# vincenthz/eccoxide

Hardware: AMD Instinct MI355X
Metric: variable-base scalarmuls/sec (batch) per GPU + achieved HBM GB/s vs roofline (higher is better)
Workload: dtype u32

## Files before the change

### __graft_entry__.py

```python
import os
import subprocess
import sys

ROOT = os.path.dirname(os.path.abspath(__file__))
if ROOT not in sys.path:
    sys.path.insert(0, ROOT)


def build() -> None:
    jobs = str(min(6, os.cpu_count() or 1))
    subprocess.check_call(["make", "-C", os.path.join(ROOT, "eccoxide_amd", "csrc"), "-j", jobs, "ARCH=gfx950"])
    subprocess.check_call(["make", "-C", os.path.join(ROOT, "oracle")])
    subprocess.check_call(["make", "-C", os.path.join(ROOT, "tests", "cpp")])
    subprocess.check_call(["make", "-C", os.path.join(ROOT, "tests", "hip")])
    subprocess.check_call(["make", "-C", os.path.join(ROOT, "tests", "hip_p256k1")])
    subprocess.check_call(["make", "-C", os.path.join(ROOT, "tests", "hip_merged")])
    import eccoxide_amd
    from eccoxide_amd import _lib

    lib = _lib.load()
    assert lib.eccx_field_bytes(eccoxide_amd.P256R1) == 32


def smoke() -> None:
    import eccoxide_amd as E
    from eccoxide_amd import workload as W
    from tests import oracle_lib

    ora = oracle_lib.load()
    with E.Engine(0) as eng:
        for curve, n in (("p256r1", 300), ("ed25519", 300)):
# ... 41 lines not shown
```

### eccoxide_amd/csrc/ufe.hpp

```cpp
#pragma once
#include "fe.hpp"

#ifndef ECCX_SOLINAS_REDUCE
#define ECCX_SOLINAS_REDUCE 1
#endif

namespace eccx {

#include "umad_chunks.inc"

__device__ __forceinline__ void smad1_k(uint64_t& acc, uint32_t a, int32_t k) {
  asm("v_mad_i64_i32 %0, vcc, %1, %2, %0" : "+v"(acc) : "v"(a), "s"(k) : "vcc");
}

__device__ __forceinline__ void smad1_v(uint64_t& acc, int32_t a, int32_t b) {
  asm("v_mad_i64_i32 %0, vcc, %1, %2, %0" : "+v"(acc) : "v"(a), "v"(b) : "vcc");
}

enum : int { UK_MONT_PP1 = 0, UK_MONT = 1, UK_MERSENNE = 2, UK_PM19 = 3 };

template <class C, int K, int V>
struct U {
  static_assert(K >= 1 && K < (1 << (32 - C::B)), "limb bound out of range (limbs must stay below 2^32)");
  static_assert(V >= 1 && V <= 4096, "value bound out of range");
  uint32_t v[C::N];
};

template <class C>
struct UB {
  static constexpr bool MONT = C::KIND == UK_MONT_PP1 || C::KIND == UK_MONT;
  static constexpr bool WRAPPED = C::KIND == UK_MERSENNE;
  static constexpr int KMAX = (1 << (32 - C::B)) - 1;
  static constexpr uint64_t COL = (uint64_t)1 << (2 * C::B);
  static constexpr bool SPARSE = C::KIND == UK_MONT_PP1 && C::SPARSE_N > 0;
  static constexpr int KKMAX = WRAPPED  ? (int)(~(uint64_t)0 / ((uint64_t)(2 * C::N - 1) * COL))
                               : SPARSE ? (int)((~(uint64_t)0 >> 1) / ((uint64_t)C::N * COL)) - 1
                                        : (int)(~(uint64_t)0 / ((uint64_t)C::N * COL)) - 1;
  static_assert(KKMAX >= 1, "limbs too wide for this many columns");
  static constexpr bool kk_ok(int k1, int k2) { return k1 * k2 <= KKMAX; }
  static constexpr int KSQ_SHIFT = WRAPPED ? 2 : 1;
  static constexpr bool ksq_ok(int k) { return k * k <= KKMAX && (k << KSQ_SHIFT) <= KMAX + 1; }
  static constexpr int vout(int v1, int v2) {
    return MONT ? (int)(((uint32_t)(v1 * v2) + C::RP - 1) / C::RP) + 1 : (C::KIND == UK_PM19 ? 2 : 3);
  }
  static constexpr int KLAZY = ksq_ok(2) ? 2 : 1;
};

template <bool KC>
struct UMacQ {
  uint32_t x[9], y[9];
  int n = 0;
  ECCX_DEV void push(uint64_t& acc, uint32_t a, uint32_t b) {
    x[n] = a;
    y[n] = b;
    if (++n == 9) flush(acc);
  }
  ECCX_DEV void flush(uint64_t& acc) {
#define ECCX_Q(i) x[i], y[i]
    if constexpr (KC) {
      switch (n) {
// ... 15 lines not shown
        case 3: umad3_v(acc, ECCX_Q(0), ECCX_Q(1), ECCX_Q(2)); break;
        case 4: umad4_v(acc, ECCX_Q(0), ECCX_Q(1), ECCX_Q(2), ECCX_Q(3)); break;
        case 5: umad5_v(acc, ECCX_Q(0), ECCX_Q(1), ECCX_Q(2), ECCX_Q(3), ECCX_Q(4)); break;
        case 6: umad6_v(acc, ECCX_Q(0), ECCX_Q(1), ECCX_Q(2), ECCX_Q(3), ECCX_Q(4), ECCX_Q(5)); break;
        case 7: umad7_v(acc, ECCX_Q(0), ECCX_Q(1), ECCX_Q(2), ECCX_Q(3), ECCX_Q(4), ECCX_Q(5), ECCX_Q(6)); break;
        case 8: umad8_v(acc, ECCX_Q(0), ECCX_Q(1), ECCX_Q(2), ECCX_Q(3), ECCX_Q(4), ECCX_Q(5), ECCX_Q(6), ECCX_Q(7)); break;
        case 9: umad9_v(acc, ECCX_Q(0), ECCX_Q(1), ECCX_Q(2), ECCX_Q(3), ECCX_Q(4), ECCX_Q(5), ECCX_Q(6), ECCX_Q(7), ECCX_Q(8)); break;
        default: break;
      }
    }
#undef ECCX_Q
    n = 0;
  }
};


template <class C, bool SQR, bool BCONST>
ECCX_DEV void u_mul_core_mont(uint32_t (&r)[C::N], const uint32_t (&a)[C::N], const uint32_t (&b)[C::N]) {
  constexpr int N = C::N;
  constexpr bool PP1 = C::KIND == UK_MONT_PP1;
  auto PR = [](int j) constexpr { return PP1 ? C::PP1[j] : C::P[j]; };
  uint32_t m[N], t[N], a2[N];
  if constexpr (SQR) {
#pragma unroll
    for (int i = 0; i < N; ++i) a2[i] = a[i] << 1;
  }
  uint64_t acc = 0;
  UMacQ<BCONST> qa;
  UMacQ<true> qm;
#pragma unroll
  for (int k = 0; k < 2 * N - 1; ++k) {
    const int lo = k < N ? 0 : k - N + 1, hi = k < N ? k : N - 1;
    if constexpr (SQR) {
#pragma unroll
      for (int i = lo; 2 * i < k; ++i) qa.push(acc, a[i], a2[k - i]);
      if ((k & 1) == 0) qa.push(acc, a[k / 2], a[k / 2]);
    } else {
#pragma unroll
      for (int i = lo; i <= hi; ++i) qa.push(acc, a[i], b[k - i]);
    }
    qa.flush(acc);
    if constexpr (UB<C>::SPARSE) {
#pragma unroll
// ... 5 lines not shown
      }
      qm.flush(acc);
#pragma unroll
      for (int t = 0; t < C::SPARSE_N; ++t) {
        const int i = k - C::SPARSE_OFF[t];
        if (i >= lo && i <= (k < N ? k - 1 : N - 1)) {
          if (C::SPARSE_SIGN[t] < 0) smad1_k(acc, m[i], -(int32_t)(1u << C::SPARSE_SHIFT[t]));
        }
      }
    } else {
#pragma unroll
      for (int i = lo; i <= (k < N ? k - 1 : N - 1); ++i) {
        if (PR(k - i) != 0) qm.push(acc, m[i], PR(k - i));
      }
      qm.flush(acc);
    }
    if (k < N) {
      if constexpr (PP1) {
        m[k] = (uint32_t)acc & C::MASK;
      } else {
        m[k] = ((uint32_t)acc * C::N0B) & C::MASK;
        umad1_k(acc, m[k], C::P[0]);
      }
    } else {
      t[k - N] = (uint32_t)acc & C::MASK;
    }
    if constexpr (UB<C>::SPARSE) acc = (uint64_t)((int64_t)acc >> C::B);
    else acc >>= C::B;
  }
  t[N - 1] = (uint32_t)acc;
// ... 138 lines not shown
  t[N - 1] = (uint32_t)acc;
#pragma unroll
  for (int i = 0; i < N; ++i) r[i] = t[i];
}

template <class C, bool NEG_SQ>
ECCX_DEV void u_mul_sub_core_pp1(uint32_t (&r)[C::N], const uint32_t (&a)[C::N], const uint32_t (&b)[C::N],
                                 const uint32_t (&c)[C::N], const uint32_t (&d)[C::N]) {
  constexpr int N = C::N;
  static_assert(C::KIND == UK_MONT_PP1 && C::SPARSE_N == 0, "p = -1 mod 2^B with p + 1 as plain digits");
  uint32_t m[N], t[N];
  int32_t nc[N];
#pragma unroll
  for (int i = 0; i < N; ++i) nc[i] = NEG_SQ ? -(int32_t)(c[i] << 1) : -(int32_t)c[i];
  uint64_t acc = 0;
  UMacQ<false> qa;
  UMacQ<true> qm;
#pragma unroll
  for (int k = 0; k < 2 * N - 1; ++k) {
    const int lo = k < N ? 0 : k - N + 1, hi = k < N ? k : N - 1;
    if (k >= N && C::P[k - N] != 0) acc += (uint64_t)C::P[k - N];
#pragma unroll
    for (int i = lo; i <= hi; ++i) qa.push(acc, a[i], b[k - i]);
    qa.flush(acc);
    if constexpr (NEG_SQ) {
#pragma unroll
      for (int i = lo; 2 * i < k; ++i) smad1_v(acc, nc[i], (int32_t)(c[k - i] << 1));
      if ((k & 1) == 0) smad1_v(acc, nc[k / 2], (int32_t)c[k / 2]);
    } else {
#pragma unroll
      for (int i = lo; i <= hi; ++i) smad1_v(acc, nc[i], (int32_t)d[k - i]);
    }
#pragma unroll
    for (int i = lo; i <= (k < N ? k - 1 : N - 1); ++i) {
      if (C::PP1[k - i] != 0) qm.push(acc, m[i], C::PP1[k - i]);
    }
    qm.flush(acc);
    if (k < N) m[k] = (uint32_t)acc & C::MASK;
    else t[k - N] = (uint32_t)acc & C::MASK;
    acc = (uint64_t)((int64_t)acc >> C::B);
  }
  acc += (uint64_t)C::P[N - 1];
  t[N - 1] = (uint32_t)acc;
#pragma unroll
  for (int i = 0; i < N; ++i) r[i] = t[i];
}

template <class C, bool SQR, bool BCONST>
ECCX_DEV void u_mul_core_mers(uint32_t (&r)[C::N], const uint32_t (&a)[C::N], const uint32_t (&b)[C::N]) {
  constexpr int N = C::N;
  constexpr int S = C::B * N - C::PBITS;
  static_assert(S >= 1 && S <= 2, "wrap factor must keep shifted limbs below 2^32");
// ... 200 lines not shown
ECCX_DEV auto u_mul_add(const U<C, K1, V1>& a, const U<C, K2, V2>& b, const U<C, K3, V3>& c, const U<C, K4, V4>& d) {
  static_assert(C::KIND == UK_MONT, "merged products are implemented for the general Montgomery fields");
  static_assert(K1 * K2 + K3 * K4 <= UB<C>::KKMAX, "two products overflow the columns: reduce an operand first");
  constexpr int VO = (int)(((uint32_t)(V1 * V2 + V3 * V4) + C::RP - 1) / C::RP) + 1;
  static_assert(VO <= 3, "result too large: reduce an operand first");
  U<C, 1, VO> r;
  u_mul2_core_mont<C>(r.v, a.v, b.v, c.v, d.v);
  return r;
}

template <class C>
struct UBS {
  static constexpr bool OK = UB<C>::SPARSE || C::KIND == UK_MONT;
  static constexpr bool DENSE = C::KIND == UK_MONT_PP1 && !UB<C>::SPARSE;
  static constexpr int KKS = (int)((~(uint64_t)0 >> 1) / ((uint64_t)C::N * UB<C>::COL)) - 1;
  static constexpr bool ks_ok(int k) { return ((uint64_t)(k + 1) << C::B) <= ((uint64_t)1 << 31); }
};

template <class C, int K1, int V1, int K2, int V2, int K3, int V3, int K4, int V4>
ECCX_DEV auto u_mul_sub(const U<C, K1, V1>& a, const U<C, K2, V2>& b, const U<C, K3, V3>& c, const U<C, K4, V4>& d) {
  static_assert(UBS<C>::OK || UBS<C>::DENSE, "implemented for the Montgomery fields with room for signed columns");
  static_assert(K1 * K2 <= UBS<C>::KKS && K3 * K4 <= UBS<C>::KKS, "a product overflows the signed columns");
  static_assert(UBS<C>::ks_ok(K3) && UBS<C>::ks_ok(K4), "negated / signed operands must stay below 2^31");
  static_assert((uint32_t)(V1 * V2) < C::RP && (uint32_t)(V3 * V4) < C::RP, "result outside (0, 3p)");
  U<C, 1, 3> r;
  if constexpr (UB<C>::SPARSE) u_mul_sub_core_sparse<C, false>(r.v, a.v, b.v, c.v, d.v);
  else if constexpr (UBS<C>::DENSE) u_mul_sub_core_pp1<C, false>(r.v, a.v, b.v, c.v, d.v);
  else u_mul_sub_core_mont<C, false>(r.v, a.v, b.v, c.v, d.v);
  return r;
}
// ... 20 lines not shown
    return r;
  }
}

template <class C, int K1, int V1>
ECCX_DEV auto u_mul_k(const U<C, K1, V1>& a, const uint32_t (&k)[C::N]) {
  if constexpr (!UB<C>::kk_ok(K1, 1) || (UB<C>::vout(V1, 1) > 3)) {
    return u_mul_k(u_reduce(a), k);
  } else {
    U<C, 1, UB<C>::vout(V1, 1)> r;
    u_mul_core<C, false, true>(r.v, a.v, k);
    return r;
  }
}

template <class C, int K1, int V1>
ECCX_DEV U<C, 1, 2> u_mul_small(const U<C, K1, V1>& a, uint32_t k) {
  static_assert(C::KIND == UK_PM19, "written for 2^255 - 19");
  constexpr int N = C::N;
  uint32_t t[N];
  uint64_t acc = 0;
#pragma unroll
  for (int i = 0; i < N; ++i) {
    umad1_v(acc, a.v[i], k);
    t[i] = (uint32_t)acc & C::MASK;
    acc >>= C::B;
  }
  u_pm_tail<C>(t, acc);
  U<C, 1, 2> r;
#pragma unroll
// ... 162 lines not shown
}

template <class C>
ECCX_DEV U<C, 1, 2> u_to_mont(const Fe<C::Sat::L>& plain) {
  if constexpr (UB<C>::MONT) return u_as<1, 2>(u_mul_k<C>(u_from_sat<C>(plain), C::R2));
  else return u_from_sat<C>(plain);
}

template <class C, int K, int V>
ECCX_DEV void u_to_canonical(Fe<C::Sat::L>& out, const U<C, K, V>& a) {
  Fe<C::Sat::L> s;
  if constexpr (UB<C>::MONT) {
    uint32_t one[C::N];
#pragma unroll
    for (int i = 0; i < C::N; ++i) one[i] = (i == 0) ? 1u : 0u;
    auto r = u_mul_k<C>(u_reduce(a), one);
    u_to_sat<C>(s, r);
  } else {
    auto r = u_reduce(u_reduce(a));
    u_to_sat<C>(s, r);
  }
  uint32_t t[C::Sat::L];
#pragma unroll
  for (int i = 0; i < C::Sat::L; ++i) t[i] = s.v[i];
  cond_sub_p<typename C::Sat>(out, t, 0u);
}

template <class C, int K, int V>
ECCX_DEV void u_to_sat_mont(Fe<C::Sat::L>& out, const U<C, K, V>& a) {
  if constexpr (UB<C>::MONT) {
    auto r = u_mul_k<C>(u_reduce(a), C::RS);
    Fe<C::Sat::L> s;
    u_to_sat<C>(s, r);
    uint32_t t[C::Sat::L];
#pragma unroll
    for (int i = 0; i < C::Sat::L; ++i) t[i] = s.v[i];
    cond_sub_p<typename C::Sat>(out, t, 0u);
  } else {
    u_to_canonical<C>(out, a);
  }
}

}
```

### eccoxide_amd/csrc/umad_chunks.inc

```
__device__ __forceinline__ void umad1_v(uint64_t& acc, uint32_t a0, uint32_t b0) {
  asm("v_mad_u64_u32 %0, vcc, %1, %2, %0\n\t"
      : "+v"(acc)
      : "v"(a0), "v"(b0)
      : "vcc");
}
__device__ __forceinline__ void umad2_v(uint64_t& acc, uint32_t a0, uint32_t b0, uint32_t a1, uint32_t b1) {
  asm("v_mad_u64_u32 %0, vcc, %1, %2, %0\n\t"
      "v_mad_u64_u32 %0, vcc, %3, %4, %0\n\t"
      : "+v"(acc)
      : "v"(a0), "v"(b0), "v"(a1), "v"(b1)
      : "vcc");
}
__device__ __forceinline__ void umad3_v(uint64_t& acc, uint32_t a0, uint32_t b0, uint32_t a1, uint32_t b1, uint32_t a2, uint32_t b2) {
  asm("v_mad_u64_u32 %0, vcc, %1, %2, %0\n\t"
      "v_mad_u64_u32 %0, vcc, %3, %4, %0\n\t"
      "v_mad_u64_u32 %0, vcc, %5, %6, %0\n\t"
      : "+v"(acc)
      : "v"(a0), "v"(b0), "v"(a1), "v"(b1), "v"(a2), "v"(b2)
      : "vcc");
}
__device__ __forceinline__ void umad4_v(uint64_t& acc, uint32_t a0, uint32_t b0, uint32_t a1, uint32_t b1, uint32_t a2, uint32_t b2, uint32_t a3, uint32_t b3) {
  asm("v_mad_u64_u32 %0, vcc, %1, %2, %0\n\t"
      "v_mad_u64_u32 %0, vcc, %3, %4, %0\n\t"
      "v_mad_u64_u32 %0, vcc, %5, %6, %0\n\t"
// ... 140 lines not shown
}
__device__ __forceinline__ void umad9_k(uint64_t& acc, uint32_t a0, uint32_t b0, uint32_t a1, uint32_t b1, uint32_t a2, uint32_t b2, uint32_t a3, uint32_t b3, uint32_t a4, uint32_t b4, uint32_t a5, uint32_t b5, uint32_t a6, uint32_t b6, uint32_t a7, uint32_t b7, uint32_t a8, uint32_t b8) {
  asm("v_mad_u64_u32 %0, vcc, %1, %2, %0\n\t"
      "v_mad_u64_u32 %0, vcc, %3, %4, %0\n\t"
      "v_mad_u64_u32 %0, vcc, %5, %6, %0\n\t"
      "v_mad_u64_u32 %0, vcc, %7, %8, %0\n\t"
      "v_mad_u64_u32 %0, vcc, %9, %10, %0\n\t"
      "v_mad_u64_u32 %0, vcc, %11, %12, %0\n\t"
      "v_mad_u64_u32 %0, vcc, %13, %14, %0\n\t"
      "v_mad_u64_u32 %0, vcc, %15, %16, %0\n\t"
      "v_mad_u64_u32 %0, vcc, %17, %18, %0\n\t"
      : "+v"(acc)
      : "v"(a0), "s"(b0), "v"(a1), "s"(b1), "v"(a2), "s"(b2), "v"(a3), "s"(b3), "v"(a4), "s"(b4), "v"(a5), "s"(b5), "v"(a6), "s"(b6), "v"(a7), "s"(b7), "v"(a8), "s"(b8)
      : "vcc");
}
```

Baseline: 73.56 million.

## Use full 32-bit Montgomery digits and fold carry into next MAD chain

For dense p+1-form Montgomery fields, the low Montgomery digits m[k] become the full low 32 bits of the accumulator instead of B-bit masked values. The high half is carried forward by a multiply-by-2^S that is fused as the first MAD of the next column's chain, which removes the separate mask, shift and carry instructions per column. New static asserts bound column overflow, and the output value bound changes. Conversion out of Montgomery form keeps the old path through a dedicated exit multiply. This trades more inline-asm variants and looser bounds for fewer ALU ops in the inner multiply.

```diff
diff --git a/__graft_entry__.py b/__graft_entry__.py
--- a/__graft_entry__.py
+++ b/__graft_entry__.py
@@ -15,6 +15,7 @@
     subprocess.check_call(["make", "-C", os.path.join(ROOT, "tests", "hip")])
     subprocess.check_call(["make", "-C", os.path.join(ROOT, "tests", "hip_p256k1")])
     subprocess.check_call(["make", "-C", os.path.join(ROOT, "tests", "hip_merged")])
+    subprocess.check_call(["make", "-C", os.path.join(ROOT, "tests", "hip_lo32")])
     import eccoxide_amd
     from eccoxide_amd import _lib
 
diff --git a/eccoxide_amd/csrc/ufe.hpp b/eccoxide_amd/csrc/ufe.hpp
--- a/eccoxide_amd/csrc/ufe.hpp
+++ b/eccoxide_amd/csrc/ufe.hpp
@@ -1,5 +1,7 @@
 #pragma once
 #include "fe.hpp"
+
+#include <type_traits>
 
 #ifndef ECCX_SOLINAS_REDUCE
 #define ECCX_SOLINAS_REDUCE 1
@@ -15,6 +17,19 @@
 
 __device__ __forceinline__ void smad1_v(uint64_t& acc, int32_t a, int32_t b) {
   asm("v_mad_i64_i32 %0, vcc, %1, %2, %0" : "+v"(acc) : "v"(a), "v"(b) : "vcc");
+}
+
+template <int S>
+__device__ __forceinline__ void ucarry_hi(uint64_t& acc) {
+  uint64_t r;
+  asm("v_mad_u64_u32 %0, vcc, %1, %2, 0" : "=&v"(r) : "v"((uint32_t)(acc >> 32)), "n"(1 << S) : "vcc");
+  acc = r;
+}
+template <int S>
+__device__ __forceinline__ void scarry_hi(uint64_t& acc) {
+  uint64_t r;
+  asm("v_mad_i64_i32 %0, vcc, %1, %2, 0" : "=&v"(r) : "v"((uint32_t)(acc >> 32)), "n"(1 << S) : "vcc");
+  acc = r;
 }
 
 enum : int { UK_MONT_PP1 = 0, UK_MONT = 1, UK_MERSENNE = 2, UK_PM19 = 3 };
@@ -41,9 +56,28 @@
   static constexpr int KSQ_SHIFT = WRAPPED ? 2 : 1;
   static constexpr bool ksq_ok(int k) { return k * k <= KKMAX && (k << KSQ_SHIFT) <= KMAX + 1; }
   static constexpr int vout(int v1, int v2) {
-    return MONT ? (int)(((uint32_t)(v1 * v2) + C::RP - 1) / C::RP) + 1 : (C::KIND == UK_PM19 ? 2 : 3);
+    return LO32   ? (int)((uint32_t)(v1 * v2) / C::RP) + 2
+           : MONT ? (int)(((uint32_t)(v1 * v2) + C::RP - 1) / C::RP) + 1
+                  : (C::KIND == UK_PM19 ? 2 : 3);
   }
   static constexpr int KLAZY = ksq_ok(2) ? 2 : 1;
+
+  static constexpr bool LO32 = C::KIND == UK_MONT_PP1 && !SPARSE;
+  static constexpr uint64_t pp1_sum() {
+    uint64_t s = 0;
+    for (int j = 0; j < C::N; ++j) s += C::PP1[j];
+    return s;
+  }
+  static_assert(!LO32 || (uint64_t)C::N * KKMAX * COL <= ~(uint64_t)0 - 0xffffffffull * pp1_sum() -
+                                                          ((uint64_t)1 << (64 - C::B)),
+                "32-bit Montgomery digits overflow the columns");
+  static constexpr int log2_rp() {
+    int l = 0;
+    while (((uint32_t)2 << l) <= C::RP) ++l;
+    return l;
+  }
+  static_assert(!LO32 || 33 + C::B * (C::N - 2) + log2_rp() + 1 <= C::B * C::N,
+                "32-bit Montgomery digits: the excess of M over R must stay below R / RP");
 };
 
 template <bool KC>
@@ -89,8 +123,64 @@
   }
 };
 
-
-template <class C, bool SQR, bool BCONST>
+template <bool KC, int S>
+struct UMacQC {
+  UMacQ<KC> q;
+  int hc = 0;
+  uint32_t h;
+  ECCX_DEV void push(uint64_t& acc, uint32_t a, uint32_t b) {
+    q.x[q.n] = a;
+    q.y[q.n] = b;
+    if (++q.n == 9) flush(acc);
+  }
+  ECCX_DEV void carry(uint64_t acc, bool sgn) {
+    h = (uint32_t)(acc >> 32);
+    hc = sgn ? 2 : 1;
+  }
+  ECCX_DEV void flush(uint64_t& acc) {
+    if (hc) flush_carry(acc);
+    else q.flush(acc);
+  }
+  ECCX_DEV void flush_carry(uint64_t& acc) {
+    static_assert(S >= 1 && S <= 6, "carry factor 2^S must be an inline constant");
+    constexpr int F = 1 << S;
+#define ECCX_Q(i) q.x[i], q.y[i]
+#define ECCX_CHUNKS(SUF)                                                                                           \
+  switch (q.n) {                                                                                                     \
+    case 1: umad1_##SUF<F>(acc, h, ECCX_Q(0)); break;                                                              \
+    case 2: umad2_##SUF<F>(acc, h, ECCX_Q(0), ECCX_Q(1)); break;                                                   \
+    case 3: umad3_##SUF<F>(acc, h, ECCX_Q(0), ECCX_Q(1), ECCX_Q(2)); break;                                        \
+    case 4: umad4_##SUF<F>(acc, h, ECCX_Q(0), ECCX_Q(1), ECCX_Q(2), ECCX_Q(3)); break;                             \
+    case 5: umad5_##SUF<F>(acc, h, ECCX_Q(0), ECCX_Q(1), ECCX_Q(2), ECCX_Q(3), ECCX_Q(4)); break;                  \
+    case 6: umad6_##SUF<F>(acc, h, ECCX_Q(0), ECCX_Q(1), ECCX_Q(2), ECCX_Q(3), ECCX_Q(4), ECCX_Q(5)); break;       \
+    case 7: umad7_##SUF<F>(acc, h, ECCX_Q(0), ECCX_Q(1), ECCX_Q(2), ECCX_Q(3), ECCX_Q(4), ECCX_Q(5), ECCX_Q(6));   \
+      break;                                                                                                       \
+    case 8:                                                                                                        \
+      umad8_##SUF<F>(acc, h, ECCX_Q(0), ECCX_Q(1), ECCX_Q(2), ECCX_Q(3), ECCX_Q(4), ECCX_Q(5), ECCX_Q(6), ECCX_Q(7)); \
+      break;                                                                                                       \
+    case 9:                                                                                                        \
+      umad9_##SUF<F>(acc, h, ECCX_Q(0), ECCX_Q(1), ECCX_Q(2), ECCX_Q(3), ECCX_Q(4), ECCX_Q(5), ECCX_Q(6), ECCX_Q(7), \
+                     ECCX_Q(8));                                                                                   \
+      break;                                                                                                       \
+    default:                                                                                                       \
+      if (hc == 2) scarry_hi<S>(acc);                                                                              \
+      else ucarry_hi<S>(acc);                                                                                      \
+      break;                                                                                                       \
+  }
+    if constexpr (KC) {
+      if (hc == 2) { ECCX_CHUNKS(ks) } else { ECCX_CHUNKS(kc) }
+    } else {
+      if (hc == 2) { ECCX_CHUNKS(vs) } else { ECCX_CHUNKS(vc) }
+    }
+#undef ECCX_CHUNKS
+#undef ECCX_Q
+    q.n = 0;
+    hc = 0;
+  }
+};
+
+
+template <class C, bool SQR, bool BCONST, bool LO32 = UB<C>::LO32>
 ECCX_DEV void u_mul_core_mont(uint32_t (&r)[C::N], const uint32_t (&a)[C::N], const uint32_t (&b)[C::N]) {
   constexpr int N = C::N;
   constexpr bool PP1 = C::KIND == UK_MONT_PP1;
@@ -101,7 +191,7 @@
     for (int i = 0; i < N; ++i) a2[i] = a[i] << 1;
   }
   uint64_t acc = 0;
-  UMacQ<BCONST> qa;
+  std::conditional_t<UB<C>::LO32, UMacQC<BCONST, 32 - C::B>, UMacQ<BCONST>> qa;
   UMacQ<true> qm;
 #pragma unroll
   for (int k = 0; k < 2 * N - 1; ++k) {
@@ -137,6 +227,13 @@
         if (PR(k - i) != 0) qm.push(acc, m[i], PR(k - i));
       }
       qm.flush(acc);
+    }
+    if constexpr (LO32) {
+      if (k < N - 1) {
+        m[k] = (uint32_t)acc;
+        qa.carry(acc, false);
+        continue;
+      }
     }
     if (k < N) {
       if constexpr (PP1) {
@@ -305,7 +402,7 @@
 #pragma unroll
   for (int i = 0; i < N; ++i) nc[i] = NEG_SQ ? -(int32_t)(c[i] << 1) : -(int32_t)c[i];
   uint64_t acc = 0;
-  UMacQ<false> qa;
+  UMacQC<false, 32 - C::B> qa;
   UMacQ<true> qm;
 #pragma unroll
   for (int k = 0; k < 2 * N - 1; ++k) {
@@ -327,6 +424,11 @@
       if (C::PP1[k - i] != 0) qm.push(acc, m[i], C::PP1[k - i]);
     }
     qm.flush(acc);
+    if (k < N - 1) {
+      m[k] = (uint32_t)acc;
+      qa.carry(acc, true);
+      continue;
+    }
     if (k < N) m[k] = (uint32_t)acc & C::MASK;
     else t[k - N] = (uint32_t)acc & C::MASK;
     acc = (uint64_t)((int64_t)acc >> C::B);
@@ -557,6 +659,9 @@
   static constexpr bool OK = UB<C>::SPARSE || C::KIND == UK_MONT;
   static constexpr bool DENSE = C::KIND == UK_MONT_PP1 && !UB<C>::SPARSE;
   static constexpr int KKS = (int)((~(uint64_t)0 >> 1) / ((uint64_t)C::N * UB<C>::COL)) - 1;
+  static_assert(!DENSE || (uint64_t)C::N * KKS * UB<C>::COL <= (~(uint64_t)0 >> 1) - 0xffffffffull * UB<C>::pp1_sum() -
+                                                                ((uint64_t)1 << C::B) - ((uint64_t)1 << (63 - C::B)),
+                "32-bit Montgomery digits overflow the signed columns");
   static constexpr bool ks_ok(int k) { return ((uint64_t)(k + 1) << C::B) <= ((uint64_t)1 << 31); }
 };
 
@@ -607,6 +712,14 @@
   }
 }
 
+template <class C>
+ECCX_DEV U<C, 1, 2> u_mul_k_exit(const U<C, 1, 3>& a, const uint32_t (&k)[C::N]) {
+  static_assert(UB<C>::MONT && UB<C>::vout(3, 1) <= 2, "Montgomery fields; a reduced operand times a constant below p");
+  U<C, 1, 2> r;
+  u_mul_core_mont<C, false, true, false>(r.v, a.v, k);
+  return r;
+}
+
 template <class C, int K1, int V1>
 ECCX_DEV U<C, 1, 2> u_mul_small(const U<C, K1, V1>& a, uint32_t k) {
   static_assert(C::KIND == UK_PM19, "written for 2^255 - 19");
@@ -799,7 +912,7 @@
     uint32_t one[C::N];
 #pragma unroll
     for (int i = 0; i < C::N; ++i) one[i] = (i == 0) ? 1u : 0u;
-    auto r = u_mul_k<C>(u_reduce(a), one);
+    auto r = u_mul_k_exit<C>(u_reduce(a), one);
     u_to_sat<C>(s, r);
   } else {
     auto r = u_reduce(u_reduce(a));
@@ -814,7 +927,7 @@
 template <class C, int K, int V>
 ECCX_DEV void u_to_sat_mont(Fe<C::Sat::L>& out, const U<C, K, V>& a) {
   if constexpr (UB<C>::MONT) {
-    auto r = u_mul_k<C>(u_reduce(a), C::RS);
+    auto r = u_mul_k_exit<C>(u_reduce(a), C::RS);
     Fe<C::Sat::L> s;
     u_to_sat<C>(s, r);
     uint32_t t[C::Sat::L];
diff --git a/eccoxide_amd/csrc/umad_chunks.inc b/eccoxide_amd/csrc/umad_chunks.inc
--- a/eccoxide_amd/csrc/umad_chunks.inc
+++ b/eccoxide_amd/csrc/umad_chunks.inc
@@ -178,3 +178,435 @@
       : "v"(a0), "s"(b0), "v"(a1), "s"(b1), "v"(a2), "s"(b2), "v"(a3), "s"(b3), "v"(a4), "s"(b4), "v"(a5), "s"(b5), "v"(a6), "s"(b6), "v"(a7), "s"(b7), "v"(a8), "s"(b8)
       : "vcc");
 }
+template <int F>
+__device__ __forceinline__ void umad1_vc(uint64_t& acc, uint32_t h, uint32_t a0, uint32_t b0) {
+  asm("v_mad_u64_u32 %0, vcc, %1, %2, 0\n\t"
+      "v_mad_u64_u32 %0, vcc, %3, %4, %0\n\t"
+      : "=&v"(acc)
+      : "v"(h), "n"(F), "v"(a0), "v"(b0)
+      : "vcc");
+}
+template <int F>
+__device__ __forceinline__ void umad2_vc(uint64_t& acc, uint32_t h, uint32_t a0, uint32_t b0, uint32_t a1, uint32_t b1) {
+  asm("v_mad_u64_u32 %0, vcc, %1, %2, 0\n\t"
+      "v_mad_u64_u32 %0, vcc, %3, %4, %0\n\t"
+      "v_mad_u64_u32 %0, vcc, %5, %6, %0\n\t"
+      : "=&v"(acc)
+      : "v"(h), "n"(F), "v"(a0), "v"(b0), "v"(a1), "v"(b1)
+      : "vcc");
+}
+template <int F>
+__device__ __forceinline__ void umad3_vc(uint64_t& acc, uint32_t h, uint32_t a0, uint32_t b0, uint32_t a1, uint32_t b1, uint32_t a2, uint32_t b2) {
+  asm("v_mad_u64_u32 %0, vcc, %1, %2, 0\n\t"
+      "v_mad_u64_u32 %0, vcc, %3, %4, %0\n\t"
+      "v_mad_u64_u32 %0, vcc, %5, %6, %0\n\t"
+      "v_mad_u64_u32 %0, vcc, %7, %8, %0\n\t"
+      : "=&v"(acc)
+      : "v"(h), "n"(F), "v"(a0), "v"(b0), "v"(a1), "v"(b1), "v"(a2), "v"(b2)
+      : "vcc");
+}
+template <int F>
+__device__ __forceinline__ void umad4_vc(uint64_t& acc, uint32_t h, uint32_t a0, uint32_t b0, uint32_t a1, uint32_t b1, uint32_t a2, uint32_t b2, uint32_t a3, uint32_t b3) {
+  asm("v_mad_u64_u32 %0, vcc, %1, %2, 0\n\t"
+      "v_mad_u64_u32 %0, vcc, %3, %4, %0\n\t"
+      "v_mad_u64_u32 %0, vcc, %5, %6, %0\n\t"
+      "v_mad_u64_u32 %0, vcc, %7, %8, %0\n\t"
+      "v_mad_u64_u32 %0, vcc, %9, %10, %0\n\t"
+      : "=&v"(acc)
+      : "v"(h), "n"(F), "v"(a0), "v"(b0), "v"(a1), "v"(b1), "v"(a2), "v"(b2), "v"(a3), "v"(b3)
+      : "vcc");
+}
+template <int F>
+__device__ __forceinline__ void umad5_vc(uint64_t& acc, uint32_t h, uint32_t a0, uint32_t b0, uint32_t a1, uint32_t b1, uint32_t a2, uint32_t b2, uint32_t a3, uint32_t b3, uint32_t a4, uint32_t b4) {
+  asm("v_mad_u64_u32 %0, vcc, %1, %2, 0\n\t"
+      "v_mad_u64_u32 %0, vcc, %3, %4, %0\n\t"
+      "v_mad_u64_u32 %0, vcc, %5, %6, %0\n\t"
+      "v_mad_u64_u32 %0, vcc, %7, %8, %0\n\t"
+      "v_mad_u64_u32 %0, vcc, %9, %10, %0\n\t"
+      "v_mad_u64_u32 %0, vcc, %11, %12, %0\n\t"
+      : "=&v"(acc)
+      : "v"(h), "n"(F), "v"(a0), "v"(b0), "v"(a1), "v"(b1), "v"(a2), "v"(b2), "v"(a3), "v"(b3), "v"(a4), "v"(b4)
+      : "vcc");
+}
+template <int F>
+__device__ __forceinline__ void umad6_vc(uint64_t& acc, uint32_t h, uint32_t a0, uint32_t b0, uint32_t a1, uint32_t b1, uint32_t a2, uint32_t b2, uint32_t a3, uint32_t b3, uint32_t a4, uint32_t b4, uint32_t a5, uint32_t b5) {
+  asm("v_mad_u64_u32 %0, vcc, %1, %2, 0\n\t"
+      "v_mad_u64_u32 %0, vcc, %3, %4, %0\n\t"
+      "v_mad_u64_u32 %0, vcc, %5, %6, %0\n\t"
+      "v_mad_u64_u32 %0, vcc, %7, %8, %0\n\t"
+      "v_mad_u64_u32 %0, vcc, %9, %10, %0\n\t"
+      "v_mad_u64_u32 %0, vcc, %11, %12, %0\n\t"
+      "v_mad_u64_u32 %0, vcc, %13, %14, %0\n\t"
+      : "=&v"(acc)
+      : "v"(h), "n"(F), "v"(a0), "v"(b0), "v"(a1), "v"(b1), "v"(a2), "v"(b2), "v"(a3), "v"(b3), "v"(a4), "v"(b4), "v"(a5), "v"(b5)
+      : "vcc");
+}
+template <int F>
+__device__ __forceinline__ void umad7_vc(uint64_t& acc, uint32_t h, uint32_t a0, uint32_t b0, uint32_t a1, uint32_t b1, uint32_t a2, uint32_t b2, uint32_t a3, uint32_t b3, uint32_t a4, uint32_t b4, uint32_t a5, uint32_t b5, uint32_t a6, uint32_t b6) {
+  asm("v_mad_u64_u32 %0, vcc, %1, %2, 0\n\t"
+      "v_mad_u64_u32 %0, vcc, %3, %4, %0\n\t"
+      "v_mad_u64_u32 %0, vcc, %5, %6, %0\n\t"
+      "v_mad_u64_u32 %0, vcc, %7, %8, %0\n\t"
+      "v_mad_u64_u32 %0, vcc, %9, %10, %0\n\t"
+      "v_mad_u64_u32 %0, vcc, %11, %12, %0\n\t"
+      "v_mad_u64_u32 %0, vcc, %13, %14, %0\n\t"
+      "v_mad_u64_u32 %0, vcc, %15, %16, %0\n\t"
+      : "=&v"(acc)
+      : "v"(h), "n"(F), "v"(a0), "v"(b0), "v"(a1), "v"(b1), "v"(a2), "v"(b2), "v"(a3), "v"(b3), "v"(a4), "v"(b4), "v"(a5), "v"(b5), "v"(a6), "v"(b6)
+      : "vcc");
+}
+template <int F>
+__device__ __forceinline__ void umad8_vc(uint64_t& acc, uint32_t h, uint32_t a0, uint32_t b0, uint32_t a1, uint32_t b1, uint32_t a2, uint32_t b2, uint32_t a3, uint32_t b3, uint32_t a4, uint32_t b4, uint32_t a5, uint32_t b5, uint32_t a6, uint32_t b6, uint32_t a7, uint32_t b7) {
+  asm("v_mad_u64_u32 %0, vcc, %1, %2, 0\n\t"
+      "v_mad_u64_u32 %0, vcc, %3, %4, %0\n\t"
+      "v_mad_u64_u32 %0, vcc, %5, %6, %0\n\t"
+      "v_mad_u64_u32 %0, vcc, %7, %8, %0\n\t"
+      "v_mad_u64_u32 %0, vcc, %9, %10, %0\n\t"
+      "v_mad_u64_u32 %0, vcc, %11, %12, %0\n\t"
+      "v_mad_u64_u32 %0, vcc, %13, %14, %0\n\t"
+      "v_mad_u64_u32 %0, vcc, %15, %16, %0\n\t"
+      "v_mad_u64_u32 %0, vcc, %17, %18, %0\n\t"
+      : "=&v"(acc)
+      : "v"(h), "n"(F), "v"(a0), "v"(b0), "v"(a1), "v"(b1), "v"(a2), "v"(b2), "v"(a3), "v"(b3), "v"(a4), "v"(b4), "v"(a5), "v"(b5), "v"(a6), "v"(b6), "v"(a7), "v"(b7)
+      : "vcc");
+}
+template <int F>
+__device__ __forceinline__ void umad9_vc(uint64_t& acc, uint32_t h, uint32_t a0, uint32_t b0, uint32_t a1, uint32_t b1, uint32_t a2, uint32_t b2, uint32_t a3, uint32_t b3, uint32_t a4, uint32_t b4, uint32_t a5, uint32_t b5, uint32_t a6, uint32_t b6, uint32_t a7, uint32_t b7, uint32_t a8, uint32_t b8) {
+  asm("v_mad_u64_u32 %0, vcc, %1, %2, 0\n\t"
+      "v_mad_u64_u32 %0, vcc, %3, %4, %0\n\t"
+      "v_mad_u64_u32 %0, vcc, %5, %6, %0\n\t"
+      "v_mad_u64_u32 %0, vcc, %7, %8, %0\n\t"
+      "v_mad_u64_u32 %0, vcc, %9, %10, %0\n\t"
+      "v_mad_u64_u32 %0, vcc, %11, %12, %0\n\t"
+      "v_mad_u64_u32 %0, vcc, %13, %14, %0\n\t"
+      "v_mad_u64_u32 %0, vcc, %15, %16, %0\n\t"
+      "v_mad_u64_u32 %0, vcc, %17, %18, %0\n\t"
+      "v_mad_u64_u32 %0, vcc, %19, %20, %0\n\t"
+      : "=&v"(acc)
+      : "v"(h), "n"(F), "v"(a0), "v"(b0), "v"(a1), "v"(b1), "v"(a2), "v"(b2), "v"(a3), "v"(b3), "v"(a4), "v"(b4), "v"(a5), "v"(b5), "v"(a6), "v"(b6), "v"(a7), "v"(b7), "v"(a8), "v"(b8)
+      : "vcc");
+}
+template <int F>
+__device__ __forceinline__ void umad1_vs(uint64_t& acc, uint32_t h, uint32_t a0, uint32_t b0) {
+  asm("v_mad_i64_i32 %0, vcc, %1, %2, 0\n\t"
+      "v_mad_u64_u32 %0, vcc, %3, %4, %0\n\t"
+      : "=&v"(acc)
+      : "v"(h), "n"(F), "v"(a0), "v"(b0)
+      : "vcc");
+}
+template <int F>
+__device__ __forceinline__ void umad2_vs(uint64_t& acc, uint32_t h, uint32_t a0, uint32_t b0, uint32_t a1, uint32_t b1) {
+  asm("v_mad_i64_i32 %0, vcc, %1, %2, 0\n\t"
+      "v_mad_u64_u32 %0, vcc, %3, %4, %0\n\t"
+      "v_mad_u64_u32 %0, vcc, %5, %6, %0\n\t"
+      : "=&v"(acc)
+      : "v"(h), "n"(F), "v"(a0), "v"(b0), "v"(a1), "v"(b1)
+      : "vcc");
+}
+template <int F>
+__device__ __forceinline__ void umad3_vs(uint64_t& acc, uint32_t h, uint32_t a0, uint32_t b0, uint32_t a1, uint32_t b1, uint32_t a2, uint32_t b2) {
+  asm("v_mad_i64_i32 %0, vcc, %1, %2, 0\n\t"
+      "v_mad_u64_u32 %0, vcc, %3, %4, %0\n\t"
+      "v_mad_u64_u32 %0, vcc, %5, %6, %0\n\t"
+      "v_mad_u64_u32 %0, vcc, %7, %8, %0\n\t"
+      : "=&v"(acc)
+      : "v"(h), "n"(F), "v"(a0), "v"(b0), "v"(a1), "v"(b1), "v"(a2), "v"(b2)
+      : "vcc");
+}
+template <int F>
+__device__ __forceinline__ void umad4_vs(uint64_t& acc, uint32_t h, uint32_t a0, uint32_t b0, uint32_t a1, uint32_t b1, uint32_t a2, uint32_t b2, uint32_t a3, uint32_t b3) {
+  asm("v_mad_i64_i32 %0, vcc, %1, %2, 0\n\t"
+      "v_mad_u64_u32 %0, vcc, %3, %4, %0\n\t"
+      "v_mad_u64_u32 %0, vcc, %5, %6, %0\n\t"
+      "v_mad_u64_u32 %0, vcc, %7, %8, %0\n\t"
+      "v_mad_u64_u32 %0, vcc, %9, %10, %0\n\t"
+      : "=&v"(acc)
+      : "v"(h), "n"(F), "v"(a0), "v"(b0), "v"(a1), "v"(b1), "v"(a2), "v"(b2), "v"(a3), "v"(b3)
+      : "vcc");
+}
+template <int F>
+__device__ __forceinline__ void umad5_vs(uint64_t& acc, uint32_t h, uint32_t a0, uint32_t b0, uint32_t a1, uint32_t b1, uint32_t a2, uint32_t b2, uint32_t a3, uint32_t b3, uint32_t a4, uint32_t b4) {
+  asm("v_mad_i64_i32 %0, vcc, %1, %2, 0\n\t"
+      "v_mad_u64_u32 %0, vcc, %3, %4, %0\n\t"
+      "v_mad_u64_u32 %0, vcc, %5, %6, %0\n\t"
+      "v_mad_u64_u32 %0, vcc, %7, %8, %0\n\t"
+      "v_mad_u64_u32 %0, vcc, %9, %10, %0\n\t"
+      "v_mad_u64_u32 %0, vcc, %11, %12, %0\n\t"
+      : "=&v"(acc)
+      : "v"(h), "n"(F), "v"(a0), "v"(b0), "v"(a1), "v"(b1), "v"(a2), "v"(b2), "v"(a3), "v"(b3), "v"(a4), "v"(b4)
+      : "vcc");
+}
+template <int F>
+__device__ __forceinline__ void umad6_vs(uint64_t& acc, uint32_t h, uint32_t a0, uint32_t b0, uint32_t a1, uint32_t b1, uint32_t a2, uint32_t b2, uint32_t a3, uint32_t b3, uint32_t a4, uint32_t b4, uint32_t a5, uint32_t b5) {
+  asm("v_mad_i64_i32 %0, vcc, %1, %2, 0\n\t"
+      "v_mad_u64_u32 %0, vcc, %3, %4, %0\n\t"
+      "v_mad_u64_u32 %0, vcc, %5, %6, %0\n\t"
+      "v_mad_u64_u32 %0, vcc, %7, %8, %0\n\t"
+      "v_mad_u64_u32 %0, vcc, %9, %10, %0\n\t"
+      "v_mad_u64_u32 %0, vcc, %11, %12, %0\n\t"
+      "v_mad_u64_u32 %0, vcc, %13, %14, %0\n\t"
+      : "=&v"(acc)
+      : "v"(h), "n"(F), "v"(a0), "v"(b0), "v"(a1), "v"(b1), "v"(a2), "v"(b2), "v"(a3), "v"(b3), "v"(a4), "v"(b4), "v"(a5), "v"(b5)
+      : "vcc");
+}
+template <int F>
+__device__ __forceinline__ void umad7_vs(uint64_t& acc, uint32_t h, uint32_t a0, uint32_t b0, uint32_t a1, uint32_t b1, uint32_t a2, uint32_t b2, uint32_t a3, uint32_t b3, uint32_t a4, uint32_t b4, uint32_t a5, uint32_t b5, uint32_t a6, uint32_t b6) {
+  asm("v_mad_i64_i32 %0, vcc, %1, %2, 0\n\t"
+      "v_mad_u64_u32 %0, vcc, %3, %4, %0\n\t"
+      "v_mad_u64_u32 %0, vcc, %5, %6, %0\n\t"
+      "v_mad_u64_u32 %0, vcc, %7, %8, %0\n\t"
+      "v_mad_u64_u32 %0, vcc, %9, %10, %0\n\t"
+      "v_mad_u64_u32 %0, vcc, %11, %12, %0\n\t"
+      "v_mad_u64_u32 %0, vcc, %13, %14, %0\n\t"
+      "v_mad_u64_u32 %0, vcc, %15, %16, %0\n\t"
+      : "=&v"(acc)
+      : "v"(h), "n"(F), "v"(a0), "v"(b0), "v"(a1), "v"(b1), "v"(a2), "v"(b2), "v"(a3), "v"(b3), "v"(a4), "v"(b4), "v"(a5), "v"(b5), "v"(a6), "v"(b6)
+      : "vcc");
+}
+template <int F>
+__device__ __forceinline__ void umad8_vs(uint64_t& acc, uint32_t h, uint32_t a0, uint32_t b0, uint32_t a1, uint32_t b1, uint32_t a2, uint32_t b2, uint32_t a3, uint32_t b3, uint32_t a4, uint32_t b4, uint32_t a5, uint32_t b5, uint32_t a6, uint32_t b6, uint32_t a7, uint32_t b7) {
+  asm("v_mad_i64_i32 %0, vcc, %1, %2, 0\n\t"
+      "v_mad_u64_u32 %0, vcc, %3, %4, %0\n\t"
+      "v_mad_u64_u32 %0, vcc, %5, %6, %0\n\t"
+      "v_mad_u64_u32 %0, vcc, %7, %8, %0\n\t"
+      "v_mad_u64_u32 %0, vcc, %9, %10, %0\n\t"
+      "v_mad_u64_u32 %0, vcc, %11, %12, %0\n\t"
+      "v_mad_u64_u32 %0, vcc, %13, %14, %0\n\t"
+      "v_mad_u64_u32 %0, vcc, %15, %16, %0\n\t"
+      "v_mad_u64_u32 %0, vcc, %17, %18, %0\n\t"
+      : "=&v"(acc)
+      : "v"(h), "n"(F), "v"(a0), "v"(b0), "v"(a1), "v"(b1), "v"(a2), "v"(b2), "v"(a3), "v"(b3), "v"(a4), "v"(b4), "v"(a5), "v"(b5), "v"(a6), "v"(b6), "v"(a7), "v"(b7)
+      : "vcc");
+}
+template <int F>
+__device__ __forceinline__ void umad9_vs(uint64_t& acc, uint32_t h, uint32_t a0, uint32_t b0, uint32_t a1, uint32_t b1, uint32_t a2, uint32_t b2, uint32_t a3, uint32_t b3, uint32_t a4, uint32_t b4, uint32_t a5, uint32_t b5, uint32_t a6, uint32_t b6, uint32_t a7, uint32_t b7, uint32_t a8, uint32_t b8) {
+  asm("v_mad_i64_i32 %0, vcc, %1, %2, 0\n\t"
+      "v_mad_u64_u32 %0, vcc, %3, %4, %0\n\t"
+      "v_mad_u64_u32 %0, vcc, %5, %6, %0\n\t"
+      "v_mad_u64_u32 %0, vcc, %7, %8, %0\n\t"
+      "v_mad_u64_u32 %0, vcc, %9, %10, %0\n\t"
+      "v_mad_u64_u32 %0, vcc, %11, %12, %0\n\t"
+      "v_mad_u64_u32 %0, vcc, %13, %14, %0\n\t"
+      "v_mad_u64_u32 %0, vcc, %15, %16, %0\n\t"
+      "v_mad_u64_u32 %0, vcc, %17, %18, %0\n\t"
+      "v_mad_u64_u32 %0, vcc, %19, %20, %0\n\t"
+      : "=&v"(acc)
+      : "v"(h), "n"(F), "v"(a0), "v"(b0), "v"(a1), "v"(b1), "v"(a2), "v"(b2), "v"(a3), "v"(b3), "v"(a4), "v"(b4), "v"(a5), "v"(b5), "v"(a6), "v"(b6), "v"(a7), "v"(b7), "v"(a8), "v"(b8)
+      : "vcc");
+}
+template <int F>
+__device__ __forceinline__ void umad1_kc(uint64_t& acc, uint32_t h, uint32_t a0, uint32_t b0) {
+  asm("v_mad_u64_u32 %0, vcc, %1, %2, 0\n\t"
+      "v_mad_u64_u32 %0, vcc, %3, %4, %0\n\t"
+      : "=&v"(acc)
+      : "v"(h), "n"(F), "v"(a0), "s"(b0)
+      : "vcc");
+}
+template <int F>
+__device__ __forceinline__ void umad2_kc(uint64_t& acc, uint32_t h, uint32_t a0, uint32_t b0, uint32_t a1, uint32_t b1) {
+  asm("v_mad_u64_u32 %0, vcc, %1, %2, 0\n\t"
+      "v_mad_u64_u32 %0, vcc, %3, %4, %0\n\t"
+      "v_mad_u64_u32 %0, vcc, %5, %6, %0\n\t"
+      : "=&v"(acc)
+      : "v"(h), "n"(F), "v"(a0), "s"(b0), "v"(a1), "s"(b1)
+      : "vcc");
+}
+template <int F>
+__device__ __forceinline__ void umad3_kc(uint64_t& acc, uint32_t h, uint32_t a0, uint32_t b0, uint32_t a1, uint32_t b1, uint32_t a2, uint32_t b2) {
+  asm("v_mad_u64_u32 %0, vcc, %1, %2, 0\n\t"
+      "v_mad_u64_u32 %0, vcc, %3, %4, %0\n\t"
+      "v_mad_u64_u32 %0, vcc, %5, %6, %0\n\t"
+      "v_mad_u64_u32 %0, vcc, %7, %8, %0\n\t"
+      : "=&v"(acc)
+      : "v"(h), "n"(F), "v"(a0), "s"(b0), "v"(a1), "s"(b1), "v"(a2), "s"(b2)
+      : "vcc");
+}
+template <int F>
+__device__ __forceinline__ void umad4_kc(uint64_t& acc, uint32_t h, uint32_t a0, uint32_t b0, uint32_t a1, uint32_t b1, uint32_t a2, uint32_t b2, uint32_t a3, uint32_t b3) {
+  asm("v_mad_u64_u32 %0, vcc, %1, %2, 0\n\t"
+      "v_mad_u64_u32 %0, vcc, %3, %4, %0\n\t"
+      "v_mad_u64_u32 %0, vcc, %5, %6, %0\n\t"
+      "v_mad_u64_u32 %0, vcc, %7, %8, %0\n\t"
+      "v_mad_u64_u32 %0, vcc, %9, %10, %0\n\t"
+      : "=&v"(acc)
+      : "v"(h), "n"(F), "v"(a0), "s"(b0), "v"(a1), "s"(b1), "v"(a2), "s"(b2), "v"(a3), "s"(b3)
+      : "vcc");
+}
+template <int F>
+__device__ __forceinline__ void umad5_kc(uint64_t& acc, uint32_t h, uint32_t a0, uint32_t b0, uint32_t a1, uint32_t b1, uint32_t a2, uint32_t b2, uint32_t a3, uint32_t b3, uint32_t a4, uint32_t b4) {
+  asm("v_mad_u64_u32 %0, vcc, %1, %2, 0\n\t"
+      "v_mad_u64_u32 %0, vcc, %3, %4, %0\n\t"
+      "v_mad_u64_u32 %0, vcc, %5, %6, %0\n\t"
+      "v_mad_u64_u32 %0, vcc, %7, %8, %0\n\t"
+      "v_mad_u64_u32 %0, vcc, %9, %10, %0\n\t"
+      "v_mad_u64_u32 %0, vcc, %11, %12, %0\n\t"
+      : "=&v"(acc)
+      : "v"(h), "n"(F), "v"(a0), "s"(b0), "v"(a1), "s"(b1), "v"(a2), "s"(b2), "v"(a3), "s"(b3), "v"(a4), "s"(b4)
+      : "vcc");
+}
+template <int F>
+__device__ __forceinline__ void umad6_kc(uint64_t& acc, uint32_t h, uint32_t a0, uint32_t b0, uint32_t a1, uint32_t b1, uint32_t a2, uint32_t b2, uint32_t a3, uint32_t b3, uint32_t a4, uint32_t b4, uint32_t a5, uint32_t b5) {
+  asm("v_mad_u64_u32 %0, vcc, %1, %2, 0\n\t"
+      "v_mad_u64_u32 %0, vcc, %3, %4, %0\n\t"
+      "v_mad_u64_u32 %0, vcc, %5, %6, %0\n\t"
+      "v_mad_u64_u32 %0, vcc, %7, %8, %0\n\t"
+      "v_mad_u64_u32 %0, vcc, %9, %10, %0\n\t"
+      "v_mad_u64_u32 %0, vcc, %11, %12, %0\n\t"
+      "v_mad_u64_u32 %0, vcc, %13, %14, %0\n\t"
+      : "=&v"(acc)
+      : "v"(h), "n"(F), "v"(a0), "s"(b0), "v"(a1), "s"(b1), "v"(a2), "s"(b2), "v"(a3), "s"(b3), "v"(a4), "s"(b4), "v"(a5), "s"(b5)
+      : "vcc");
+}
+template <int F>
+__device__ __forceinline__ void umad7_kc(uint64_t& acc, uint32_t h, uint32_t a0, uint32_t b0, uint32_t a1, uint32_t b1, uint32_t a2, uint32_t b2, uint32_t a3, uint32_t b3, uint32_t a4, uint32_t b4, uint32_t a5, uint32_t b5, uint32_t a6, uint32_t b6) {
+  asm("v_mad_u64_u32 %0, vcc, %1, %2, 0\n\t"
+      "v_mad_u64_u32 %0, vcc, %3, %4, %0\n\t"
+      "v_mad_u64_u32 %0, vcc, %5, %6, %0\n\t"
+      "v_mad_u64_u32 %0, vcc, %7, %8, %0\n\t"
+      "v_mad_u64_u32 %0, vcc, %9, %10, %0\n\t"
+      "v_mad_u64_u32 %0, vcc, %11, %12, %0\n\t"
+      "v_mad_u64_u32 %0, vcc, %13, %14, %0\n\t"
+      "v_mad_u64_u32 %0, vcc, %15, %16, %0\n\t"
+      : "=&v"(acc)
+      : "v"(h), "n"(F), "v"(a0), "s"(b0), "v"(a1), "s"(b1), "v"(a2), "s"(b2), "v"(a3), "s"(b3), "v"(a4), "s"(b4), "v"(a5), "s"(b5), "v"(a6), "s"(b6)
+      : "vcc");
+}
+template <int F>
+__device__ __forceinline__ void umad8_kc(uint64_t& acc, uint32_t h, uint32_t a0, uint32_t b0, uint32_t a1, uint32_t b1, uint32_t a2, uint32_t b2, uint32_t a3, uint32_t b3, uint32_t a4, uint32_t b4, uint32_t a5, uint32_t b5, uint32_t a6, uint32_t b6, uint32_t a7, uint32_t b7) {
+  asm("v_mad_u64_u32 %0, vcc, %1, %2, 0\n\t"
+      "v_mad_u64_u32 %0, vcc, %3, %4, %0\n\t"
+      "v_mad_u64_u32 %0, vcc, %5, %6, %0\n\t"
+      "v_mad_u64_u32 %0, vcc, %7, %8, %0\n\t"
+      "v_mad_u64_u32 %0, vcc, %9, %10, %0\n\t"
+      "v_mad_u64_u32 %0, vcc, %11, %12, %0\n\t"
+      "v_mad_u64_u32 %0, vcc, %13, %14, %0\n\t"
+      "v_mad_u64_u32 %0, vcc, %15, %16, %0\n\t"
+      "v_mad_u64_u32 %0, vcc, %17, %18, %0\n\t"
+      : "=&v"(acc)
+      : "v"(h), "n"(F), "v"(a0), "s"(b0), "v"(a1), "s"(b1), "v"(a2), "s"(b2), "v"(a3), "s"(b3), "v"(a4), "s"(b4), "v"(a5), "s"(b5), "v"(a6), "s"(b6), "v"(a7), "s"(b7)
+      : "vcc");
+}
+template <int F>
+__device__ __forceinline__ void umad9_kc(uint64_t& acc, uint32_t h, uint32_t a0, uint32_t b0, uint32_t a1, uint32_t b1, uint32_t a2, uint32_t b2, uint32_t a3, uint32_t b3, uint32_t a4, uint32_t b4, uint32_t a5, uint32_t b5, uint32_t a6, uint32_t b6, uint32_t a7, uint32_t b7, uint32_t a8, uint32_t b8) {
+  asm("v_mad_u64_u32 %0, vcc, %1, %2, 0\n\t"
+      "v_mad_u64_u32 %0, vcc, %3, %4, %0\n\t"
+      "v_mad_u64_u32 %0, vcc, %5, %6, %0\n\t"
+      "v_mad_u64_u32 %0, vcc, %7, %8, %0\n\t"
+      "v_mad_u64_u32 %0, vcc, %9, %10, %0\n\t"
+      "v_mad_u64_u32 %0, vcc, %11, %12, %0\n\t"
+      "v_mad_u64_u32 %0, vcc, %13, %14, %0\n\t"
+      "v_mad_u64_u32 %0, vcc, %15, %16, %0\n\t"
+      "v_mad_u64_u32 %0, vcc, %17, %18, %0\n\t"
+      "v_mad_u64_u32 %0, vcc, %19, %20, %0\n\t"
+      : "=&v"(acc)
+      : "v"(h), "n"(F), "v"(a0), "s"(b0), "v"(a1), "s"(b1), "v"(a2), "s"(b2), "v"(a3), "s"(b3), "v"(a4), "s"(b4), "v"(a5), "s"(b5), "v"(a6), "s"(b6), "v"(a7), "s"(b7), "v"(a8), "s"(b8)
+      : "vcc");
+}
+template <int F>
+__device__ __forceinline__ void umad1_ks(uint64_t& acc, uint32_t h, uint32_t a0, uint32_t b0) {
+  asm("v_mad_i64_i32 %0, vcc, %1, %2, 0\n\t"
+      "v_mad_u64_u32 %0, vcc, %3, %4, %0\n\t"
+      : "=&v"(acc)
+      : "v"(h), "n"(F), "v"(a0), "s"(b0)
+      : "vcc");
+}
+template <int F>
+__device__ __forceinline__ void umad2_ks(uint64_t& acc, uint32_t h, uint32_t a0, uint32_t b0, uint32_t a1, uint32_t b1) {
+  asm("v_mad_i64_i32 %0, vcc, %1, %2, 0\n\t"
+      "v_mad_u64_u32 %0, vcc, %3, %4, %0\n\t"
+      "v_mad_u64_u32 %0, vcc, %5, %6, %0\n\t"
+      : "=&v"(acc)
+      : "v"(h), "n"(F), "v"(a0), "s"(b0), "v"(a1), "s"(b1)
+      : "vcc");
+}
+template <int F>
+__device__ __forceinline__ void umad3_ks(uint64_t& acc, uint32_t h, uint32_t a0, uint32_t b0, uint32_t a1, uint32_t b1, uint32_t a2, uint32_t b2) {
+  asm("v_mad_i64_i32 %0, vcc, %1, %2, 0\n\t"
+      "v_mad_u64_u32 %0, vcc, %3, %4, %0\n\t"
+      "v_mad_u64_u32 %0, vcc, %5, %6, %0\n\t"
+      "v_mad_u64_u32 %0, vcc, %7, %8, %0\n\t"
+      : "=&v"(acc)
+      : "v"(h), "n"(F), "v"(a0), "s"(b0), "v"(a1), "s"(b1), "v"(a2), "s"(b2)
+      : "vcc");
+}
+template <int F>
+__device__ __forceinline__ void umad4_ks(uint64_t& acc, uint32_t h, uint32_t a0, uint32_t b0, uint32_t a1, uint32_t b1, uint32_t a2, uint32_t b2, uint32_t a3, uint32_t b3) {
+  asm("v_mad_i64_i32 %0, vcc, %1, %2, 0\n\t"
+      "v_mad_u64_u32 %0, vcc, %3, %4, %0\n\t"
+      "v_mad_u64_u32 %0, vcc, %5, %6, %0\n\t"
+      "v_mad_u64_u32 %0, vcc, %7, %8, %0\n\t"
+      "v_mad_u64_u32 %0, vcc, %9, %10, %0\n\t"
+      : "=&v"(acc)
+      : "v"(h), "n"(F), "v"(a0), "s"(b0), "v"(a1), "s"(b1), "v"(a2), "s"(b2), "v"(a3), "s"(b3)
+      : "vcc");
+}
+template <int F>
+__device__ __forceinline__ void umad5_ks(uint64_t& acc, uint32_t h, uint32_t a0, uint32_t b0, uint32_t a1, uint32_t b1, uint32_t a2, uint32_t b2, uint32_t a3, uint32_t b3, uint32_t a4, uint32_t b4) {
+  asm("v_mad_i64_i32 %0, vcc, %1, %2, 0\n\t"
+      "v_mad_u64_u32 %0, vcc, %3, %4, %0\n\t"
+      "v_mad_u64_u32 %0, vcc, %5, %6, %0\n\t"
+      "v_mad_u64_u32 %0, vcc, %7, %8, %0\n\t"
+      "v_mad_u64_u32 %0, vcc, %9, %10, %0\n\t"
+      "v_mad_u64_u32 %0, vcc, %11, %12, %0\n\t"
+      : "=&v"(acc)
+      : "v"(h), "n"(F), "v"(a0), "s"(b0), "v"(a1), "s"(b1), "v"(a2), "s"(b2), "v"(a3), "s"(b3), "v"(a4), "s"(b4)
+      : "vcc");
+}
+template <int F>
+__device__ __forceinline__ void umad6_ks(uint64_t& acc, uint32_t h, uint32_t a0, uint32_t b0, uint32_t a1, uint32_t b1, uint32_t a2, uint32_t b2, uint32_t a3, uint32_t b3, uint32_t a4, uint32_t b4, uint32_t a5, uint32_t b5) {
+  asm("v_mad_i64_i32 %0, vcc, %1, %2, 0\n\t"
+      "v_mad_u64_u32 %0, vcc, %3, %4, %0\n\t"
+      "v_mad_u64_u32 %0, vcc, %5, %6, %0\n\t"
+      "v_mad_u64_u32 %0, vcc, %7, %8, %0\n\t"
+      "v_mad_u64_u32 %0, vcc, %9, %10, %0\n\t"
+      "v_mad_u64_u32 %0, vcc, %11, %12, %0\n\t"
+      "v_mad_u64_u32 %0, vcc, %13, %14, %0\n\t"
+      : "=&v"(acc)
+      : "v"(h), "n"(F), "v"(a0), "s"(b0), "v"(a1), "s"(b1), "v"(a2), "s"(b2), "v"(a3), "s"(b3), "v"(a4), "s"(b4), "v"(a5), "s"(b5)
+      : "vcc");
+}
+template <int F>
+__device__ __forceinline__ void umad7_ks(uint64_t& acc, uint32_t h, uint32_t a0, uint32_t b0, uint32_t a1, uint32_t b1, uint32_t a2, uint32_t b2, uint32_t a3, uint32_t b3, uint32_t a4, uint32_t b4, uint32_t a5, uint32_t b5, uint32_t a6, uint32_t b6) {
+  asm("v_mad_i64_i32 %0, vcc, %1, %2, 0\n\t"
+      "v_mad_u64_u32 %0, vcc, %3, %4, %0\n\t"
+      "v_mad_u64_u32 %0, vcc, %5, %6, %0\n\t"
+      "v_mad_u64_u32 %0, vcc, %7, %8, %0\n\t"
+      "v_mad_u64_u32 %0, vcc, %9, %10, %0\n\t"
+      "v_mad_u64_u32 %0, vcc, %11, %12, %0\n\t"
+      "v_mad_u64_u32 %0, vcc, %13, %14, %0\n\t"
+      "v_mad_u64_u32 %0, vcc, %15, %16, %0\n\t"
+      : "=&v"(acc)
+      : "v"(h), "n"(F), "v"(a0), "s"(b0), "v"(a1), "s"(b1), "v"(a2), "s"(b2), "v"(a3), "s"(b3), "v"(a4), "s"(b4), "v"(a5), "s"(b5), "v"(a6), "s"(b6)
+      : "vcc");
+}
+template <int F>
+__device__ __forceinline__ void umad8_ks(uint64_t& acc, uint32_t h, uint32_t a0, uint32_t b0, uint32_t a1, uint32_t b1, uint32_t a2, uint32_t b2, uint32_t a3, uint32_t b3, uint32_t a4, uint32_t b4, uint32_t a5, uint32_t b5, uint32_t a6, uint32_t b6, uint32_t a7, uint32_t b7) {
+  asm("v_mad_i64_i32 %0, vcc, %1, %2, 0\n\t"
+      "v_mad_u64_u32 %0, vcc, %3, %4, %0\n\t"
+      "v_mad_u64_u32 %0, vcc, %5, %6, %0\n\t"
+      "v_mad_u64_u32 %0, vcc, %7, %8, %0\n\t"
+      "v_mad_u64_u32 %0, vcc, %9, %10, %0\n\t"
+      "v_mad_u64_u32 %0, vcc, %11, %12, %0\n\t"
+      "v_mad_u64_u32 %0, vcc, %13, %14, %0\n\t"
+      "v_mad_u64_u32 %0, vcc, %15, %16, %0\n\t"
+      "v_mad_u64_u32 %0, vcc, %17, %18, %0\n\t"
+      : "=&v"(acc)
+      : "v"(h), "n"(F), "v"(a0), "s"(b0), "v"(a1), "s"(b1), "v"(a2), "s"(b2), "v"(a3), "s"(b3), "v"(a4), "s"(b4), "v"(a5), "s"(b5), "v"(a6), "s"(b6), "v"(a7), "s"(b7)
+      : "vcc");
+}
+template <int F>
+__device__ __forceinline__ void umad9_ks(uint64_t& acc, uint32_t h, uint32_t a0, uint32_t b0, uint32_t a1, uint32_t b1, uint32_t a2, uint32_t b2, uint32_t a3, uint32_t b3, uint32_t a4, uint32_t b4, uint32_t a5, uint32_t b5, uint32_t a6, uint32_t b6, uint32_t a7, uint32_t b7, uint32_t a8, uint32_t b8) {
+  asm("v_mad_i64_i32 %0, vcc, %1, %2, 0\n\t"
+      "v_mad_u64_u32 %0, vcc, %3, %4, %0\n\t"
+      "v_mad_u64_u32 %0, vcc, %5, %6, %0\n\t"
+      "v_mad_u64_u32 %0, vcc, %7, %8, %0\n\t"
+      "v_mad_u64_u32 %0, vcc, %9, %10, %0\n\t"
+      "v_mad_u64_u32 %0, vcc, %11, %12, %0\n\t"
+      "v_mad_u64_u32 %0, vcc, %13, %14, %0\n\t"
+      "v_mad_u64_u32 %0, vcc, %15, %16, %0\n\t"
+      "v_mad_u64_u32 %0, vcc, %17, %18, %0\n\t"
+      "v_mad_u64_u32 %0, vcc, %19, %20, %0\n\t"
+      : "=&v"(acc)
+      : "v"(h), "n"(F), "v"(a0), "s"(b0), "v"(a1), "s"(b1), "v"(a2), "s"(b2), "v"(a3), "s"(b3), "v"(a4), "s"(b4), "v"(a5), "s"(b5), "v"(a6), "s"(b6), "v"(a7), "s"(b7), "v"(a8), "s"(b8)
+      : "vcc");
+}
```

Measured after the change: 75.30 million (median of 6 runs). 2.4% higher.
